# cr1m5onk1ng/text_similarity

Hardware: AMD Instinct MI355X
Metric: sentences/sec encoded + Mpairs/sec cosine top-k @ N=1M d=384 (higher is better)
Workload: dtype bf16 encoder / f16 selection / fp32 scores

## Files before the change

text_similarity_amd/csrc/encoder.hip:

```cpp
#include <math.h>
#include <cmath>

#include <stdlib.h>
#include <string.h>

#include <vector>

#include <type_traits>
#include <utility>

#include "common.h"
#include "gemm_pp.h"

namespace tsim {

__device__ __forceinline__ int64_t packed_off(int64_t t, int f, int W) {
    return ((t >> 5) * (W >> 3) + (f >> 3)) * 256 + (t & 31) * 8 + (f & 7);
}
__device__ __forceinline__ int64_t group_off(int64_t t, int g, int W, int packed) {
    return packed ? packed_off(t, 8 * g, W) * 2 : (t * W + 8 * g) * 2;
}

template <int VPL, bool TYPED = false>
__global__ __launch_bounds__(256) void embed_ln_kernel(const int32_t *__restrict__ ids,
                                                       const int32_t *__restrict__ pos,
                                                       const float *__restrict__ word,
                                                       const float *__restrict__ pos_emb,
                                                       const float *__restrict__ type_tab,
                                                       const float *__restrict__ gamma,
                                                       const float *__restrict__ beta, float eps, int T, int H,
                                                       bf16_t *__restrict__ out, int vocab, int max_pos,
                                                       const int32_t *__restrict__ col, int max_len,
                                                       int *__restrict__ err_flags,
                                                       const int32_t *__restrict__ tok_type = nullptr, int n_types = 0) {
    const int lane = threadIdx.x & 63;
    const int t = blockIdx.x * 4 + (threadIdx.x >> 6);
    if (t >= T) return;
    int id = ids[t], ps = pos[t];
    int ty = 0;
    if constexpr (TYPED) ty = tok_type[t];
    int bad = 0;
    if (id < 0 || id >= vocab) { bad |= TSIM_ENC_ERR_TOKEN_ID; id = id < 0 ? 0 : vocab - 1; }
    if (ps < 0 || ps >= max_pos) { bad |= TSIM_ENC_ERR_POSITION; ps = ps < 0 ? 0 : max_pos - 1; }
    if (col[t] >= max_len || col[t] < 0) bad |= TSIM_ENC_ERR_MAX_LEN;
    if constexpr (TYPED) {
        if (ty < 0 || ty >= n_types) { bad |= TSIM_ENC_ERR_TOKEN_TYPE; ty = ty < 0 ? 0 : n_types - 1; }
    }
    if (bad && lane == 0) atomicOr(err_flags, bad);
    const float *w = word + (int64_t)id * H;
    const float *p = pos_emb + (int64_t)ps * H;
    const float *type_row = TYPED ? type_tab + (int64_t)ty * H : type_tab;
    float v[VPL], pv[VPL], tv[VPL];
#pragma unroll
    for (int i = 0; i < VPL; ++i) {
        v[i] = w[lane + i * 64];
        pv[i] = p[lane + i * 64];
    }
    if (type_row) {
#pragma unroll
        for (int i = 0; i < VPL; ++i) tv[i] = type_row[lane + i * 64];
    }
    float s = 0.f;
#pragma unroll
    for (int i = 0; i < VPL; ++i) {
        float a = v[i];
        if (type_row) a += tv[i];
        a += pv[i];
        v[i] = a;
        s += a;
    }
    const float mean = wave_sum(s) / (float)H;
    float q = 0.f;
#pragma unroll
    for (int i = 0; i < VPL; ++i) {
        const float dlt = v[i] - mean;
        q = fmaf(dlt, dlt, q);
    }
    const float rstd = 1.0f / sqrtf(wave_sum(q) / (float)H + eps);
#pragma unroll
    for (int i = 0; i < VPL; ++i) {
        const int j = lane + i * 64;
        out[(int64_t)t * H + j] = f32_to_bf16((v[i] - mean) * rstd * gamma[j] + beta[j]);
    }
}

enum { EPI_BIAS = 0, EPI_GELU = 1, EPI_RES_LN = 2 };

template <int BM, int BN, int BK, int WAVES_M, int WAVES_N, int NST = 2>
constexpr int gemm_lds_bytes() {
    return NST * (BM + BN) * BK * 2;
}

template <int BM, int BN, int BK, int WAVES_M, int WAVES_N, int EPI, int NST = 2>
__global__ __launch_bounds__(WAVES_M *WAVES_N * 64) void gemm_bf16_kernel(
    const bf16_t *__restrict__ X, const bf16_t *__restrict__ W, const float *__restrict__ bias,
    const bf16_t *__restrict__ res, const float *__restrict__ gamma, const float *__restrict__ beta, float eps,
    bf16_t *__restrict__ out, int M, int N, int K, int mtiles, int ntiles, const bf16_t *__restrict__ Wimg, int xpacked,
    int respacked, int opacked) {
    constexpr int NW = WAVES_M * WAVES_N;
    constexpr int TM = BM / WAVES_M, TN = BN / WAVES_N, MT = TM / 32, NT = TN / 32;
    constexpr int RB = BK * 2;
    constexpr int CPR = RB / 16;
    constexpr int RPS = 256 / RB;
    constexpr int X_BYTES = BM * RB, W_BYTES = BN * RB, STAGE = X_BYTES + W_BYTES;
    constexpr int PIECES = STAGE / 1024, XPIECES = X_BYTES / 1024;
    constexpr int KSTEPS = BK / 16;
    static_assert(TM % 32 == 0 && TN % 32 == 0 && X_BYTES % 1024 == 0 && W_BYTES % 1024 == 0, "tile shape");
    static_assert(NST == 2 || PIECES % NW == 0, "a deep ring needs equal DMA counts per wave");
    constexpr int PPW = (PIECES + NW - 1) / NW;
    extern __shared__ __attribute__((aligned(16))) char smem[];

    const int lane = threadIdx.x & 63;
    const int wave = __builtin_amdgcn_readfirstlane(threadIdx.x >> 6);
    const int wm = wave / WAVES_N, wn = wave % WAVES_N;
    const int r = lane & 31, h = lane >> 5;

    const int b = blockIdx.x, xcd = b & 7, jj = b >> 3;
    const int nt_id = jj % ntiles;
    const int mt_id = (jj / ntiles) * 8 + xcd;
// ... 583 lines not shown
    for (; kt + LR_NST <= nk; kt += LR_NST)
        ff_static_for(std::make_integer_sequence<int, LR_NST>{}, [&](auto sc) __attribute__((always_inline)) {
            do_tile(kt + decltype(sc)::value, sc);
        });
    ff_static_for(std::make_integer_sequence<int, LR_NST - 1>{}, [&](auto sc) __attribute__((always_inline)) {
        if (kt + decltype(sc)::value < nk) do_tile(kt + decltype(sc)::value, sc);
    });
    wait_vmcnt<0>();

    const int64_t m = m0 + wave * 32 + r;
    const bool live = m < M;
    const int64_t mr = live ? m : M - 1;
    const uint32_t ro = (uint32_t)group_off(mr, h, N, respacked), rgs = (uint32_t)group_off(0, 1, N, respacked);
#pragma unroll
    for (int t = 0; t < 12; ++t)
#pragma unroll
        for (int gq = 0; gq < 4; gq += 2) {
            const uint4 o = *reinterpret_cast<const uint4 *>(reinterpret_cast<const char *>(res) + (ro + (4 * t + gq) * rgs));
            auto s0 = __builtin_amdgcn_permlane32_swap(o.x, o.z, false, false);
            auto s1 = __builtin_amdgcn_permlane32_swap(o.y, o.w, false, false);
            const uint32_t a0 = s0[0], c0 = s0[1], a1 = s1[0], c1 = s1[1];
            acc[t][4 * gq + 0] += __uint_as_float(a0 << 16);
            acc[t][4 * gq + 1] += __uint_as_float(a0 & 0xffff0000u);
            acc[t][4 * gq + 2] += __uint_as_float(a1 << 16);
            acc[t][4 * gq + 3] += __uint_as_float(a1 & 0xffff0000u);
            acc[t][4 * gq + 4] += __uint_as_float(c0 << 16);
            acc[t][4 * gq + 5] += __uint_as_float(c0 & 0xffff0000u);
            acc[t][4 * gq + 6] += __uint_as_float(c1 << 16);
            acc[t][4 * gq + 7] += __uint_as_float(c1 & 0xffff0000u);
        }
    float mean, rstd;
#pragma unroll
    for (int pass = 0; pass < 2; ++pass) {
        float tot = 0.f;
#pragma unroll
        for (int w = 0; w < 4; ++w) {
            float sg = 0.f;
#pragma unroll
            for (int t = 3 * w; t < 3 * w + 3; ++t)
#pragma unroll
                for (int q = 0; q < 16; ++q) {
                    if (pass == 0) {
                        sg += acc[t][q];
                    } else {
                        const float dlt = acc[t][q] - mean;
                        sg = fmaf(dlt, dlt, sg);
                    }
                }
            sg += __shfl_xor(sg, 32, 64);
            tot += sg;
        }
        if (pass == 0)
            mean = tot / (float)N;
        else
            rstd = 1.0f / sqrtf(tot / (float)N + eps);
    }
    const uint32_t oo = (uint32_t)group_off(m, h, N, opacked), ogs = (uint32_t)group_off(0, 1, N, opacked);
#pragma unroll
    for (int t = 0; t < 12; ++t) {
        uint32_t pk[8];
#pragma unroll
        for (int gq = 0; gq < 4; ++gq) {
            const int n = 32 * t + 8 * gq + 4 * h;
            const f32x4 gv = *reinterpret_cast<const f32x4 *>(gamma + n), bv = *reinterpret_cast<const f32x4 *>(beta + n);
            const float o0 = fmaf((acc[t][4 * gq + 0] - mean) * rstd, gv[0], bv[0]);
            const float o1 = fmaf((acc[t][4 * gq + 1] - mean) * rstd, gv[1], bv[1]);
            const float o2 = fmaf((acc[t][4 * gq + 2] - mean) * rstd, gv[2], bv[2]);
            const float o3 = fmaf((acc[t][4 * gq + 3] - mean) * rstd, gv[3], bv[3]);
            pk[2 * gq] = pack_bf16x2(o0, o1);
            pk[2 * gq + 1] = pack_bf16x2(o2, o3);
        }
#pragma unroll
        for (int gq = 0; gq < 4; gq += 2) {
            auto s0 = __builtin_amdgcn_permlane32_swap(pk[2 * gq], pk[2 * gq + 2], false, false);
            auto s1w = __builtin_amdgcn_permlane32_swap(pk[2 * gq + 1], pk[2 * gq + 3], false, false);
            if (live)
                *reinterpret_cast<uint4 *>(reinterpret_cast<char *>(out) + (oo + (4 * t + gq) * ogs)) = make_uint4(s0[0], s1w[0], s0[1], s1w[1]);
        }
    }
}

template <int DH, bool REL, bool PK = false>
__global__ __launch_bounds__(256) __attribute__((amdgpu_waves_per_eu(DH <= 32 ? 6 : 4))) void attention_kernel(const bf16_t *__restrict__ qkv,
                                                        const int32_t *__restrict__ cu, const int32_t *__restrict__ col,
                                                        const float *__restrict__ relb, int relw, int H,
                                                        int heads, float scale, bf16_t *__restrict__ ctx, int B, int xcd_map) {
    constexpr int KS = DH / 16;
    constexpr int OT = (DH + 31) / 32;
    constexpr int ROWB = DH * 2 < 64 ? 64 : DH * 2;
    __shared__ __attribute__((aligned(16))) char vimg[4 * 32 * ROWB];
    typedef __attribute__((ext_vector_type(4))) short s16x4;
    const int lane = threadIdx.x & 63;
    const int wave = __builtin_amdgcn_readfirstlane(threadIdx.x >> 6);
    int seq = blockIdx.x;
    if (xcd_map) {
        seq = (blockIdx.x & 7) * (gridDim.x >> 3) + (blockIdx.x >> 3);
        if (seq >= B) return;
    }
    const int head = blockIdx.y * 4 + wave, qb = blockIdx.z;
    const int t0 = cu[seq], S = cu[seq + 1] - t0;
    if (qb * 32 >= S || head >= heads) return;
    const int r = lane & 31, h = lane >> 5;
    const int64_t H3 = 3 * (int64_t)H;
    const int qi = qb * 32 + r;
    const int tq = t0 + (qi < S ? qi : S - 1);

    bf16x8 qf[KS];
    {
        const bf16_t *qp = PK ? qkv + packed_off(tq, head * DH + 8 * h, (int)H3) : qkv + tq * H3 + head * DH + 8 * h;
#pragma unroll
        for (int s = 0; s < KS; ++s) {
            qf[s] = *reinterpret_cast<const bf16x8 *>(qp + (PK ? 2 * 256 : 16) * s);
        }
    }
    const int qcol = REL ? col[tq] : 0;
    f32x16 o[OT];
#pragma unroll
    for (int ob = 0; ob < OT; ++ob)
#pragma unroll
        for (int g = 0; g < 16; ++g) o[ob][g] = 0.f;
    float m = -INFINITY, l = 0.f;

    for (int k0 = 0; k0 < S; k0 += 32) {
        const int kr = k0 + r;
        const int tk = t0 + (kr < S ? kr : S - 1);
        f32x16 sc;
#pragma unroll
        for (int g = 0; g < 16; ++g) sc[g] = 0.f;
        constexpr int CH = DH / 16;
        uint4 vr[CH];
        {
            const bf16_t *kp = PK ? qkv + packed_off(tk, H + head * DH + 8 * h, (int)H3) : qkv + tk * H3 + H + head * DH + 8 * h;
            const bf16_t *vsrc = PK ? qkv + packed_off(tk, 2 * H + head * DH + h * (DH / 2), (int)H3)
                                    : qkv + tk * H3 + 2 * H + head * DH + h * (DH / 2);
            bf16x8 kf[KS];
#pragma unroll
            for (int s = 0; s < KS; ++s) kf[s] = *reinterpret_cast<const bf16x8 *>(kp + (PK ? 2 * 256 : 16) * s);
#pragma unroll
            for (int c = 0; c < CH; ++c) vr[c] = *reinterpret_cast<const uint4 *>(vsrc + (PK ? 256 : 8) * c);
#pragma unroll
            for (int s = 0; s < KS; ++s) sc = __builtin_amdgcn_mfma_f32_32x32x16_bf16(kf[s], qf[s], sc, 0, 0, 0);
        }
        float bm = -INFINITY;
#pragma unroll
        for (int g = 0; g < 16; ++g) {
            const int key = k0 + (g & 3) + 8 * (g >> 2) + 4 * h;
            float v = sc[g] * scale;
            if (REL) {
                const int kc = col[t0 + (key < S ? key : S - 1)];
                v += relb[head * relw + (kc - qcol) + (relw >> 1)];
            }
            v = key < S ? v : -INFINITY;
            sc[g] = v;
            bm = fmaxf(bm, v);
        }
        bm = fmaxf(bm, __shfl_xor(bm, 32, 64));
        const float mn = fmaxf(m, bm);
        const float corr = __expf(m - mn);
        float ps = 0.f;
#pragma unroll
        for (int g = 0; g < 16; ++g) {
            sc[g] = __expf(sc[g] - mn);
            ps += sc[g];
        }
        ps += __shfl_xor(ps, 32, 64);
        l = l * corr + ps;
        m = mn;
#pragma unroll
        for (int ob = 0; ob < OT; ++ob)
#pragma unroll
            for (int g = 0; g < 16; ++g) o[ob][g] *= corr;
        bf16x8 pf[2];
#pragma unroll
        for (int s = 0; s < 2; ++s)
#pragma unroll
            for (int j = 0; j < 8; ++j) pf[s][j] = (__bf16)sc[8 * s + j];
        {
            char *vrow = vimg + wave * (32 * ROWB) + r * ROWB + h * DH;
#pragma unroll
            for (int c = 0; c < CH; ++c) *reinterpret_cast<uint4 *>(vrow + 16 * c) = vr[c];
        }
        __builtin_amdgcn_wave_barrier();
#pragma unroll
        for (int ob = 0; ob < OT; ++ob) {
// ... 391 lines not shown
                    const double de = (double)(float)hv - (double)y[j] * inv;
                    r2 = fma(de, de, r2);
                }
                unit[(int64_t)b * ld_unit + j] = hv;
            }
            if (rho_max) {
                const float rho = rho_round_up(sqrt(wave_sum_f64(r2)));
                if (lane == 0) rho_publish(rho_max, rho);
            }
        }
    }
}

static int dense_rows_launch(const float *x, int B, int d_in, const float *w, const float *bias, int d_out, int act, int normalize,
                             float *out, unit_t *unit, int ld_unit, float *rho_max, hipStream_t st) {
    if (B <= 0) return TSIM_OK;
    const dim3 grid((unsigned)((B + DN_ROWS - 1) / DN_ROWS));
    const size_t lds = (size_t)DN_ROWS * d_out * sizeof(float);
#define DENSE(NT) hipLaunchKernelGGL(dense_rows_kernel<NT>, grid, dim3(64 * DN_WAVES), lds, st, x, B, d_in, w, bias, d_out, act, normalize, out, unit, ld_unit, rho_max)
    const int nt = ((d_out + 15) / 16 + DN_WAVES - 1) / DN_WAVES;
    if (nt <= 1) DENSE(1); else if (nt <= 2) DENSE(2); else if (nt <= 3) DENSE(3); else if (nt <= 4) DENSE(4);
    else if (nt <= 6) DENSE(6); else DENSE(8);
#undef DENSE
    TSIM_HIP_CHECK(hipGetLastError());
    return TSIM_OK;
}

static int dense_check(int d_in, int d_out, int act, const float *w) {
    TSIM_REQUIRE(d_in >= 8 && d_in <= DN_MAX && d_in % 8 == 0, "dense: d_in=%d outside [8, %d] or not a multiple of 8", d_in, DN_MAX);
    TSIM_REQUIRE(d_out >= 8 && d_out <= DN_MAX && d_out % 8 == 0, "dense: d_out=%d outside [8, %d] or not a multiple of 8", d_out,
                 DN_MAX);
    TSIM_REQUIRE(w || d_out == d_in, "dense: without a weight matrix d_out (%d) must equal d_in (%d)", d_out, d_in);
    TSIM_REQUIRE(act == TSIM_ACT_IDENTITY || act == TSIM_ACT_TANH, "dense: unknown activation %d (TSIM_ACT_IDENTITY, TSIM_ACT_TANH)",
                 act);
    TSIM_REQUIRE(((uintptr_t)w & 15) == 0, "dense: the weight matrix must be 16-byte aligned");
    return TSIM_OK;
}

static uint16_t host_f32_to_bf16(float f) {
    uint32_t u;
    memcpy(&u, &f, 4);
    if ((u & 0x7fffffffu) > 0x7f800000u) return (uint16_t)((u >> 16) | 0x40);
    u += 0x7fffu + ((u >> 16) & 1u);
    return (uint16_t)(u >> 16);
}

struct DevBuf {
    void *p = nullptr;
    ~DevBuf() {
        if (p) (void)hipFree(p);
    }
};

}

using namespace tsim;

struct tsim_encoder {
    tsim_encoder_config cfg;
    int Tp = 0;
    float *word = nullptr, *pos = nullptr, *type0 = nullptr, *emb_g = nullptr, *emb_b = nullptr, *relb = nullptr;
    int relw = 0;
    int n_types = 0;
    float *head_wpT = nullptr, *head_bp = nullptr, *head_wc = nullptr, *head_bc = nullptr;
    int n_labels = 0;
    int head_act = TSIM_ACT_TANH;
    struct Layer {
        bf16_t *wqkv, *wo, *w1, *w2;
        bf16_t *pqkv = nullptr, *po = nullptr;
        bf16_t *lo = nullptr, *l2 = nullptr;
        bf16_t *lo32 = nullptr, *l232 = nullptr;
        uint8_t *qqkv = nullptr, *qo = nullptr, *q1 = nullptr, *q2 = nullptr;
        uint8_t *sqkv = nullptr, *so = nullptr, *s1 = nullptr, *s2 = nullptr;
        float *bqkv, *bo, *b1, *b2, *g1, *be1, *g2, *be2;
    };
    std::vector<Layer> layers;
    std::vector<void *> allocs;
    bf16_t *x0 = nullptr, *x1 = nullptr, *qkv = nullptr, *ctx = nullptr, *h1 = nullptr;
    float *ybuf = nullptr;
    float *lnimg = nullptr;
    float *head_x = nullptr;
    uint8_t *aq = nullptr, *as = nullptr, *hq = nullptr, *hs = nullptr;
    int *err_flags = nullptr;
};

namespace tsim {

static int dev_alloc(tsim_encoder *e, size_t bytes, void **out) {
    void *p = nullptr;
    hipError_t err = hipMalloc(&p, bytes);
    if (err != hipSuccess) return fail(TSIM_ENOMEM, "hipMalloc(%zu) failed: %s", bytes, hipGetErrorString(err));
    e->allocs.push_back(p);
    *out = p;
    return TSIM_OK;
}

static int upload_f32(tsim_encoder *e, const float *h, size_t n, float **out) {
    int rc = dev_alloc(e, n * 4, (void **)out);
    if (rc) return rc;
    TSIM_HIP_CHECK(hipMemcpy(*out, h, n * 4, hipMemcpyHostToDevice));
    return TSIM_OK;
}

static int upload_bf16(tsim_encoder *e, const std::vector<const float *> &parts, size_t n_each, bf16_t **out) {
    std::vector<uint16_t> tmp(n_each * parts.size());
    for (size_t p = 0; p < parts.size(); ++p)
        for (size_t i = 0; i < n_each; ++i) tmp[p * n_each + i] = host_f32_to_bf16(parts[p][i]);
    int rc = dev_alloc(e, tmp.size() * 2, (void **)out);
    if (rc) return rc;
    TSIM_HIP_CHECK(hipMemcpy(*out, tmp.data(), tmp.size() * 2, hipMemcpyHostToDevice));
    return TSIM_OK;
}

static uint8_t host_f32_to_e4m3(float v) {
    const uint8_t sign = std::signbit(v) ? 0x80 : 0;
    const double a = std::fabs((double)v);
    if (a == 0.0) return sign;
    int exp;
    const double mant = std::frexp(a, &exp);
    long byte;
    if (a >= std::ldexp(1.0, -6))
        byte = ((long)(exp - 1 + 7) << 3) + std::lrint((mant * 2.0 - 1.0) * 8.0);
    else
        byte = std::lrint(std::ldexp(a, 9));
    if (byte > 0x7e) byte = 0x7e;
    return (uint8_t)byte | sign;
}

static int upload_mxfp8(tsim_encoder *e, const std::vector<const float *> &parts, size_t n_rows, size_t K, uint8_t **q,
                        uint8_t **sc) {
    const size_t rows = n_rows * parts.size(), nb = K / 32;
    std::vector<uint8_t> hq(rows * K), hs(rows * nb);
    for (size_t p = 0; p < parts.size(); ++p)
        for (size_t r = 0; r < n_rows; ++r)
            for (size_t b = 0; b < nb; ++b) {
                const float *src = parts[p] + r * K + b * 32;
                float amax = 0.f;
                for (int i = 0; i < 32; ++i) amax = std::fmax(amax, std::fabs(src[i]));
                int sexp = 0;
                if (amax > 0.f) {
                    int ex;
                    (void)std::frexp((double)amax, &ex);
                    sexp = ex - 1 - 8;
                    sexp = sexp < -127 ? -127 : (sexp > 127 ? 127 : sexp);
                }
                uint8_t *dst = hq.data() + (p * n_rows + r) * K + b * 32;
                for (int i = 0; i < 32; ++i) {
                    double y = std::ldexp((double)src[i], -sexp);
                    y = y > 448.0 ? 448.0 : (y < -448.0 ? -448.0 : y);
                    dst[i] = host_f32_to_e4m3((float)y);
                }
                hs[(p * n_rows + r) * nb + b] = (uint8_t)(sexp + 127);
            }
    int rc = dev_alloc(e, hq.size(), (void **)q);
    if (rc) return rc;
    if ((rc = dev_alloc(e, hs.size(), (void **)sc))) return rc;
    TSIM_HIP_CHECK(hipMemcpy(*q, hq.data(), hq.size(), hipMemcpyHostToDevice));
    TSIM_HIP_CHECK(hipMemcpy(*sc, hs.data(), hs.size(), hipMemcpyHostToDevice));
    return TSIM_OK;
}

static int mpnet_bucket(int rel, int num_buckets) {
    int ret = 0;
    int n = -rel;
    const int nb = num_buckets / 2;
    if (n < 0) {
// ... 390 lines not shown
    }
    e->layers.resize(L);
    for (int l = 0; l < L; ++l) {
        const tsim_layer_weights_host &lw = w->layers[l];
        tsim_encoder::Layer &d = e->layers[l];
        if ((rc = upload_bf16(e, {lw.wq, lw.wk, lw.wv}, (size_t)H * H, &d.wqkv))) return bail(rc);
        if ((rc = upload_bf16(e, {lw.wo}, (size_t)H * H, &d.wo))) return bail(rc);
        if ((rc = upload_bf16(e, {lw.w1}, (size_t)F * H, &d.w1))) return bail(rc);
        if ((rc = upload_bf16(e, {lw.w2}, (size_t)H * F, &d.w2))) return bail(rc);
        if (mx) {
            if ((rc = upload_mxfp8(e, {lw.wq, lw.wk, lw.wv}, H, H, &d.qqkv, &d.sqkv))) return bail(rc);
            if ((rc = upload_mxfp8(e, {lw.wo}, H, H, &d.qo, &d.so))) return bail(rc);
            if ((rc = upload_mxfp8(e, {lw.w1}, F, H, &d.q1, &d.s1))) return bail(rc);
            if ((rc = upload_mxfp8(e, {lw.w2}, H, F, &d.q2, &d.s2))) return bail(rc);
        }
        auto repack = [&](const void *src, int n_rows, int kbytes, void **dst) {
            int r2 = dev_alloc(e, (size_t)n_rows * kbytes, dst);
            return r2 ? r2 : pack_w(src, *dst, n_rows, kbytes, gemm_pp_tile_width(n_rows), nullptr);
        };
        if (mx) {
            void *t;
            if ((rc = repack(d.qqkv, 3 * H, H, &t))) return bail(rc); d.qqkv = (uint8_t *)t;
            if ((rc = repack(d.qo, H, H, &t))) return bail(rc); d.qo = (uint8_t *)t;
            if ((rc = repack(d.q1, F, H, &t))) return bail(rc); d.q1 = (uint8_t *)t;
            if ((rc = repack(d.q2, H, F, &t))) return bail(rc); d.q2 = (uint8_t *)t;
        } else if (H >= 512 && H % 256 == 0 && gemm_pp_supported(H, H) && gemm_pp_supported(F, H) && gemm_pp_supported(H, F)) {
            if ((rc = repack(d.wqkv, 3 * H, H * 2, (void **)&d.pqkv))) return bail(rc);
            if ((rc = repack(d.wo, H, H * 2, (void **)&d.po))) return bail(rc);
        }
        if (!mx && H == 384 && F % 64 == 0) {
            if ((rc = dev_alloc(e, (size_t)H * H * 2, (void **)&d.lo))) return bail(rc);
            if ((rc = dev_alloc(e, (size_t)H * F * 2, (void **)&d.l2))) return bail(rc);
            hipLaunchKernelGGL(pack_gemm_w_kernel, dim3((unsigned)((H * H / 8 + 255) / 256)), dim3(256), 0, 0,
                               reinterpret_cast<const uint4 *>(d.wo), reinterpret_cast<uint4 *>(d.lo), 384, 64, H);
            hipLaunchKernelGGL(pack_gemm_w_kernel, dim3((unsigned)((H * F / 8 + 255) / 256)), dim3(256), 0, 0,
                               reinterpret_cast<const uint4 *>(d.w2), reinterpret_cast<uint4 *>(d.l2), 384, 64, F);
            if ((rc = dev_alloc(e, (size_t)H * H * 2, (void **)&d.lo32))) return bail(rc);
            if ((rc = dev_alloc(e, (size_t)H * F * 2, (void **)&d.l232))) return bail(rc);
            hipLaunchKernelGGL(pack_frag_w_kernel, dim3((unsigned)((H * H / 8 + 255) / 256)), dim3(256), 0, 0,
                               reinterpret_cast<const uint4 *>(d.wo), reinterpret_cast<uint4 *>(d.lo32), 384, H);
            hipLaunchKernelGGL(pack_frag_w_kernel, dim3((unsigned)((H * F / 8 + 255) / 256)), dim3(256), 0, 0,
                               reinterpret_cast<const uint4 *>(d.w2), reinterpret_cast<uint4 *>(d.l232), 384, F);
            if (hipGetLastError() != hipSuccess) return bail(fail(TSIM_EHIP, "LayerNorm GEMM weight packing failed"));
        }
        std::vector<float> bq(3 * (size_t)H);
        memcpy(bq.data(), lw.bq, H * 4);
        memcpy(bq.data() + H, lw.bk, H * 4);
        memcpy(bq.data() + 2 * H, lw.bv, H * 4);
        if ((rc = upload_f32(e, bq.data(), bq.size(), &d.bqkv))) return bail(rc);
        if ((rc = upload_f32(e, lw.bo, H, &d.bo))) return bail(rc);
        if ((rc = upload_f32(e, lw.b1, F, &d.b1))) return bail(rc);
        if ((rc = upload_f32(e, lw.b2, H, &d.b2))) return bail(rc);
        if ((rc = upload_f32(e, lw.ln1_g, H, &d.g1))) return bail(rc);
        if ((rc = upload_f32(e, lw.ln1_b, H, &d.be1))) return bail(rc);
        if ((rc = upload_f32(e, lw.ln2_g, H, &d.g2))) return bail(rc);
        if ((rc = upload_f32(e, lw.ln2_b, H, &d.be2))) return bail(rc);
    }
    const size_t Tp = e->Tp;
    struct { bf16_t **p; size_t n; } acts[] = {{&e->x0, Tp * H}, {&e->x1, Tp * H}, {&e->qkv, Tp * 3 * H},
                                               {&e->ctx, Tp * H}, {&e->h1, Tp * F}};
    for (auto &a : acts) {
        if ((rc = dev_alloc(e, a.n * 2, (void **)a.p))) return bail(rc);
        if (hipMemset(*a.p, 0, a.n * 2) != hipSuccess) return bail(fail(TSIM_EHIP, "hipMemset failed"));
    }
    if (H >= 512 && H % 256 == 0 && gemm_pp_supported(H, H)) {
        if ((rc = dev_alloc(e, Tp * H * 4, (void **)&e->ybuf))) return bail(rc);
        if (hipMemset(e->ybuf, 0, Tp * H * 4) != hipSuccess) return bail(fail(TSIM_EHIP, "hipMemset failed"));
    }
    if (!mx && H == 384 && F % 64 == 0) {
        const size_t blocks = (Tp + 31) / 32 < (size_t)LS_MAX_BLOCKS ? (Tp + 31) / 32 : (size_t)LS_MAX_BLOCKS;
        const size_t bytes = blocks * 4 * 12 * 64 * 16;
        if ((rc = dev_alloc(e, bytes, (void **)&e->lnimg))) return bail(rc);
        if (hipMemset(e->lnimg, 0, bytes) != hipSuccess) return bail(fail(TSIM_EHIP, "hipMemset failed"));
    }
    if ((size_t)cfg->max_seqs * H * 4 > Tp * 3 * H * 2 && (rc = dev_alloc(e, (size_t)cfg->max_seqs * H * 4, (void **)&e->head_x)))
        return bail(rc);
    if (mx) {
        struct { uint8_t **p; size_t n; } qb[] = {{&e->aq, Tp * H}, {&e->as, Tp * H / 32}, {&e->hq, Tp * F}, {&e->hs, Tp * F / 32}};
        for (auto &a : qb) {
            if ((rc = dev_alloc(e, a.n, (void **)a.p))) return bail(rc);
            if (hipMemset(*a.p, 0, a.n) != hipSuccess) return bail(fail(TSIM_EHIP, "hipMemset failed"));
        }
    }
    if ((rc = dev_alloc(e, 256, (void **)&e->err_flags))) return bail(rc);
    if (hipMemset(e->err_flags, 0, 256) != hipSuccess) return bail(fail(TSIM_EHIP, "hipMemset failed"));
    if (hipDeviceSynchronize() != hipSuccess) return bail(fail(TSIM_EHIP, "sync after upload failed"));
    *out = e;
    return TSIM_OK;
}

extern "C" int tsim_encoder_error_flags(tsim_encoder *e, int32_t *flags_host, void *stream) {
    TSIM_REQUIRE(e && flags_host, "encoder_error_flags: null pointer");
    hipStream_t st = reinterpret_cast<hipStream_t>(stream);
    TSIM_HIP_CHECK(hipMemcpyAsync(flags_host, e->err_flags, 4, hipMemcpyDeviceToHost, st));
    TSIM_HIP_CHECK(hipMemsetAsync(e->err_flags, 0, 4, st));
    TSIM_HIP_CHECK(hipStreamSynchronize(st));
    return TSIM_OK;
}

extern "C" int tsim_quantize_mxfp8(const void *x_bf16, int64_t rows, int K, void *q_out, void *scale_out, void *stream) {
    TSIM_REQUIRE(x_bf16 && q_out && scale_out, "quantize_mxfp8: null pointer");
    TSIM_REQUIRE(rows >= 0 && K > 0, "quantize_mxfp8: bad shape rows=%lld K=%d", (long long)rows, K);
    return quant_mx(static_cast<const bf16_t *>(x_bf16), rows, K, static_cast<uint8_t *>(q_out),
                    static_cast<uint8_t *>(scale_out), reinterpret_cast<hipStream_t>(stream));
}

extern "C" int tsim_gemm_mxfp8(const void *xq, const void *xs, const void *wq, const void *ws, const float *bias,
                               float *out_f32, int M, int N, int K, void *stream) {
    TSIM_REQUIRE(xq && xs && wq && ws && bias && out_f32, "gemm_mxfp8: null pointer");
    TSIM_REQUIRE(M >= 0 && N > 0 && K > 0, "gemm_mxfp8: bad shape M=%d N=%d K=%d", M, N, K);
    return gemm_pp_mx(PP_EPI_F32, static_cast<const uint8_t *>(xq), static_cast<const uint8_t *>(xs),
                      static_cast<const uint8_t *>(wq), 0, static_cast<const uint8_t *>(ws), bias, out_f32, nullptr, M, N, K,
                      reinterpret_cast<hipStream_t>(stream));
}

#ifdef TSIM_PP_STAMPS
extern "C" int tsim_debug_xr_stamps(unsigned long long *out16, int reset) {
    if (hipMemcpyFromSymbol(out16, HIP_SYMBOL(tsim::g_xr_stamps), 128) != hipSuccess) return 1;
    if (reset) { unsigned long long z[16] = {0}; if (hipMemcpyToSymbol(HIP_SYMBOL(tsim::g_xr_stamps), z, 128) != hipSuccess) return 1; }
    return 0;
}
#endif

extern "C" void tsim_encoder_destroy(tsim_encoder *e) {
    if (!e) return;
    for (void *p : e->allocs) (void)hipFree(p);
    delete e;
}

extern "C" int tsim_encoder_set_token_types(tsim_encoder *e, const float *type_emb_host, int32_t n_types) {
    TSIM_REQUIRE(e && type_emb_host, "encoder_set_token_types: null pointer");
    TSIM_REQUIRE(e->cfg.arch != TSIM_ARCH_MPNET, "encoder_set_token_types: BERT only (MPNet has no token-type table)");
    TSIM_REQUIRE(n_types >= 1, "encoder_set_token_types: n_types=%d < 1", n_types);
    float *tab = nullptr;
    if (int rc = upload_f32(e, type_emb_host, (size_t)n_types * e->cfg.hidden, &tab)) return rc;
    e->type0 = tab;
    e->n_types = n_types;
    return TSIM_OK;
}

extern "C" int tsim_encoder_set_cls_head(tsim_encoder *e, const float *pool_w_host, const float *pool_b_host,
                                         const float *cls_w_host, const float *cls_b_host, int32_t num_labels) {
    return tsim_encoder_set_cls_head_act(e, pool_w_host, pool_b_host, cls_w_host, cls_b_host, num_labels, TSIM_ACT_TANH);
}

extern "C" int tsim_encoder_set_cls_head_act(tsim_encoder *e, const float *pool_w_host, const float *pool_b_host,
                                             const float *cls_w_host, const float *cls_b_host, int32_t num_labels, int32_t act) {
    TSIM_REQUIRE(e && pool_w_host && pool_b_host && cls_w_host && cls_b_host, "encoder_set_cls_head: null pointer");
    TSIM_REQUIRE(e->cfg.arch != TSIM_ARCH_MPNET, "encoder_set_cls_head: BERT only");
    TSIM_REQUIRE(act == TSIM_ACT_TANH || act == TSIM_ACT_RELU, "encoder_set_cls_head: activation %d (TSIM_ACT_TANH, TSIM_ACT_RELU)", act);
    TSIM_REQUIRE(num_labels >= 1 && num_labels <= CLS_MAX_LABELS, "encoder_set_cls_head: num_labels=%d outside [1, %d]", num_labels,
                 CLS_MAX_LABELS);
    const int H = e->cfg.hidden;
    TSIM_REQUIRE(H % 64 == 0 && H <= CLS_WIDE_H, "encoder_set_cls_head: hidden=%d unsupported", H);
    std::vector<float> wT((size_t)H * H);
    for (int o = 0; o < H; ++o)
        for (int k = 0; k < H; ++k) wT[(size_t)k * H + o] = pool_w_host[(size_t)o * H + k];
    int rc;
    if ((rc = upload_f32(e, wT.data(), wT.size(), &e->head_wpT))) return rc;
    if ((rc = upload_f32(e, pool_b_host, H, &e->head_bp))) return rc;
    if ((rc = upload_f32(e, cls_w_host, (size_t)num_labels * H, &e->head_wc))) return rc;
    if ((rc = upload_f32(e, cls_b_host, num_labels, &e->head_bc))) return rc;
    e->n_labels = num_labels;
    e->head_act = act;
    return TSIM_OK;
}

extern "C" int tsim_encoder_forward(tsim_encoder *e, const int32_t *tok_ids, const int32_t *tok_pos,
                                    const int32_t *tok_col, const int32_t *cu_seqlens, int32_t T, int32_t B,
                                    int32_t max_len, float *pooled_f32, void *unit_bf16, int ld_unit, float *unit_rho_max,
                                    void *last_hidden_bf16, void *stream) {
    return tsim_encoder_forward_ex(e, tok_ids, nullptr, tok_pos, tok_col, cu_seqlens, T, B, max_len, pooled_f32, unit_bf16, ld_unit,
                                   unit_rho_max, last_hidden_bf16, nullptr, stream);
}

extern "C" int tsim_encoder_forward_ex(tsim_encoder *e, const int32_t *tok_ids, const int32_t *tok_type, const int32_t *tok_pos,
                                       const int32_t *tok_col, const int32_t *cu_seqlens, int32_t T, int32_t B,
                                       int32_t max_len, float *pooled_f32, void *unit_bf16, int ld_unit, float *unit_rho_max,
                                       void *last_hidden_bf16, float *logits_f32, void *stream) {
    TSIM_REQUIRE(e && cu_seqlens && (T == 0 || (tok_ids && tok_pos)), "encoder_forward: null pointer");
    TSIM_REQUIRE(!tok_type || e->n_types > 0, "encoder_forward: tok_type given but no token-type table was set "
                 "(tsim_encoder_set_token_types)");
    TSIM_REQUIRE(!logits_f32 || e->n_labels > 0, "encoder_forward: logits requested but no classification head was set "
                 "(tsim_encoder_set_cls_head)");
    TSIM_REQUIRE(T >= 0 && B >= 0 && T <= e->cfg.max_tokens && B <= e->cfg.max_seqs,
                 "encoder_forward: T=%d B=%d exceed capacity (%d tokens, %d sequences)", T, B, e->cfg.max_tokens, e->cfg.max_seqs);
    const int pos_span = max_len + (e->cfg.arch != TSIM_ARCH_BERT ? e->cfg.pad_id + 1 : 0);
    TSIM_REQUIRE(max_len >= 0 && pos_span <= e->cfg.max_pos,
                 "encoder_forward: sequences of %d tokens need position rows up to %d, the table has %d", max_len, pos_span - 1,
                 e->cfg.max_pos);
    TSIM_REQUIRE(!unit_bf16 || ld_unit >= e->cfg.hidden, "encoder_forward: ld_unit < hidden");
    TSIM_REQUIRE(!unit_bf16 || e->cfg.hidden <= 768, "encoder_forward: unit rows need a width <= 768 (got %d)", e->cfg.hidden);
    if (B == 0) return TSIM_OK;
    hipStream_t st = reinterpret_cast<hipStream_t>(stream);
    const tsim_encoder_config &c = e->cfg;
    const int H = c.hidden, F = c.ffn, dh = H / c.heads;
    const bool mx = c.weight_dtype == TSIM_W_MXFP8;
    int rc;
    if (T > 0) {
        const unsigned g = (unsigned)((T + 3) / 4);
        const int32_t *colp = tok_col ? tok_col : tok_pos;
        const int col_limit = tok_col || c.arch == TSIM_ARCH_BERT ? max_len : c.max_pos;
#define EMBED(V) hipLaunchKernelGGL(embed_ln_kernel<V>, dim3(g), dim3(256), 0, st, tok_ids, tok_pos, e->word, e->pos, e->type0, e->emb_g, e->emb_b, c.ln_eps, T, H, e->x0, c.vocab, c.max_pos, colp, col_limit, e->err_flags, nullptr, 0)
#define EMBED_T(V) hipLaunchKernelGGL((embed_ln_kernel<V, true>), dim3(g), dim3(256), 0, st, tok_ids, tok_pos, e->word, e->pos, e->type0, e->emb_g, e->emb_b, c.ln_eps, T, H, e->x0, c.vocab, c.max_pos, colp, col_limit, e->err_flags, tok_type, e->n_types)
        if (tok_type) {
            if (H == 64) EMBED_T(1); else if (H == 384) EMBED_T(6); else if (H == 768) EMBED_T(12); else EMBED_T(16);
        } else if (H == 64) EMBED(1); else if (H == 384) EMBED(6); else if (H == 768) EMBED(12); else EMBED(16);
#undef EMBED_T
#undef EMBED
        TSIM_HIP_CHECK(hipGetLastError());
        const float scale = 1.0f / sqrtf((float)dh);
        const bool rel = c.arch == TSIM_ARCH_MPNET;
        const bool pk = !mx && !rel && use_packed_layout(H, F);
        const int32_t *col = rel ? (tok_col ? tok_col : tok_pos) : nullptr;
        const int qblocks = (max_len + 31) / 32 > 0 ? (max_len + 31) / 32 : 1;
        const dim3 agrid((unsigned)(((B + 7) / 8) * 8), (unsigned)((c.heads + 3) / 4), (unsigned)qblocks);
        for (int l = 0; l < c.num_layers; ++l) {
            const tsim_encoder::Layer &L = e->layers[l];
            const bool x0pk = pk && l > 0, x0pk_next = pk && l + 1 < c.num_layers;
            if (mx) {
                if (l == 0 && (rc = quant_mx(e->x0, T, H, e->aq, e->as, st))) return rc;
                if ((rc = gemm_pp_mx(PP_EPI_BIAS, e->aq, e->as, L.qqkv, 1, L.sqkv, L.bqkv, e->qkv, nullptr, T, 3 * H, H, st))) return rc;
            } else if (pk) {
                rc = x0pk ? gemm_xres2<EPI_BIAS, true, true>(e->x0, L.wqkv, L.bqkv, e->qkv, T, 3 * H, st)
                          : gemm_xres2<EPI_BIAS, true>(e->x0, L.wqkv, L.bqkv, e->qkv, T, 3 * H, st);
                if (rc) return rc;
            } else if ((rc = gemm_plain<EPI_BIAS>(e->x0, L.wqkv, L.pqkv, L.bqkv, e->qkv, T, 3 * H, H, st))) return rc;
#define ATT(D)                                                                                                 \
    do {                                                                                                       \
        if (rel)                                                                                               \
            hipLaunchKernelGGL((attention_kernel<D, true>), agrid, dim3(256), 0, st, e->qkv, cu_seqlens, col,  \
                               e->relb, e->relw, H, c.heads, scale, e->ctx, B, 1);                                         \
        else if (pk)                                                                                           \
            hipLaunchKernelGGL((attention_kernel<D, false, true>), agrid, dim3(256), 0, st, e->qkv, cu_seqlens, col, \
                               e->relb, e->relw, H, c.heads, scale, e->ctx, B, 1);                                         \
        else                                                                                                   \
            hipLaunchKernelGGL((attention_kernel<D, false>), agrid, dim3(256), 0, st, e->qkv, cu_seqlens, col, \
                               e->relb, e->relw, H, c.heads, scale, e->ctx, B, 1);                                         \
    } while (0)
            if (dh == 16) ATT(16); else if (dh == 32) ATT(32); else ATT(64);
#undef ATT
            TSIM_HIP_CHECK(hipGetLastError());
            if (mx) {
                if ((rc = quant_mx(e->ctx, T, H, e->aq, e->as, st))) return rc;
                if ((rc = gemm_pp_mx(PP_EPI_F32, e->aq, e->as, L.qo, 1, L.so, L.bo, e->ybuf, nullptr, T, H, H, st))) return rc;
                if ((rc = res_ln_rows(e->ybuf, e->x0, L.g1, L.be1, c.ln_eps, e->x1, e->aq, e->as, T, H, st))) return rc;
                if ((rc = gemm_pp_mx(PP_EPI_GELU_MX, e->aq, e->as, L.q1, 1, L.s1, L.b1, e->hq, e->hs, T, F, H, st))) return rc;
                if ((rc = gemm_pp_mx(PP_EPI_F32, e->hq, e->hs, L.q2, 1, L.s2, L.b2, e->ybuf, nullptr, T, H, F, st))) return rc;
                if ((rc = res_ln_rows(e->ybuf, e->x1, L.g2, L.be2, c.ln_eps, e->x0, e->aq, e->as, T, H, st))) return rc;
                continue;
            }
            if ((rc = gemm_res_ln(e->ctx, L.wo, L.po, L.bo, e->x0, L.g1, L.be1, c.ln_eps, e->x1, T, H, H, e->ybuf, st, L.lo, L.lo32, false, e->lnimg, x0pk, pk))) return rc;
            if (pk) {
                if ((rc = gemm_xres2<EPI_GELU, true, true>(e->x1, L.w1, L.b1, e->h1, T, F, st))) return rc;
            } else if ((rc = gemm_plain<EPI_GELU>(e->x1, L.w1, nullptr, L.b1, e->h1, T, F, H, st))) return rc;
            if ((rc = gemm_res_ln(e->h1, L.w2, nullptr, L.b2, e->x1, L.g2, L.be2, c.ln_eps, e->x0, T, H, F, e->ybuf, st, L.l2, L.l232, pk, e->lnimg, pk, x0pk_next))) return rc;
        }
        if (last_hidden_bf16)
            TSIM_HIP_CHECK(hipMemcpyAsync(last_hidden_bf16, e->x0, (size_t)T * H * 2, hipMemcpyDeviceToDevice, st));
    }
    if (pooled_f32 || unit_bf16) {
        const unsigned g = (unsigned)((B + 3) / 4);
#define POOL(V) hipLaunchKernelGGL(pool_packed_kernel<V>, dim3(g), dim3(256), 0, st, e->x0, cu_seqlens, B, H, pooled_f32, (unit_t *)unit_bf16, ld_unit, unit_bf16 ? unit_rho_max : nullptr)
        if (H % 8 != 0 || H > 1024 || (unit_bf16 && ld_unit % 8 != 0))
            return fail(TSIM_EUNSUPPORTED, "encoder: pooling needs a hidden size that is a multiple of 8, at most 1024 (got %d)", H);
        if (((uintptr_t)pooled_f32 | (uintptr_t)unit_bf16) & 15)
            return fail(TSIM_EINVAL, "encoder: pooled / unit outputs must be 16-byte aligned");
        if (H <= 512) POOL(1); else POOL(2);
#undef POOL
        TSIM_HIP_CHECK(hipGetLastError());
    }
    if (logits_f32) {
        const dim3 cgrid((unsigned)((B + CLS_ROWS - 1) / CLS_ROWS)), cblock((unsigned)H);
#define CLS_WIDE(MAXH, ACT)                                                                                       \
    hipLaunchKernelGGL((cls_head_wide_kernel<MAXH, ACT>), cgrid, cblock, 0, st, e->x0, cu_seqlens, B, H, e->head_wpT, \
                       e->head_bp, e->head_wc, e->head_bc, e->n_labels, logits_f32)
        if (e->head_act == TSIM_ACT_RELU) {
            if (H <= CLS_MAX_H) CLS_WIDE(CLS_MAX_H, TSIM_ACT_RELU); else CLS_WIDE(CLS_WIDE_H, TSIM_ACT_RELU);
        } else if (H <= CLS_MAX_H) {
            hipLaunchKernelGGL(cls_head_kernel, cgrid, cblock, 0, st, e->x0, cu_seqlens,
                               B, H, e->head_wpT, e->head_bp, e->head_wc, e->head_bc, e->n_labels, logits_f32);
        } else CLS_WIDE(CLS_WIDE_H, TSIM_ACT_TANH);
#undef CLS_WIDE
        TSIM_HIP_CHECK(hipGetLastError());
    }
    return TSIM_OK;
}

extern "C" int tsim_encoder_forward_head(tsim_encoder *e, const int32_t *tok_ids, const int32_t *tok_type, const int32_t *tok_pos,
                                         const int32_t *tok_col, const int32_t *cu_seqlens, int32_t T, int32_t B, int32_t max_len,
                                         const tsim_sentence_head *head, float *emb_f32, void *unit_f16, int ld_unit,
                                         float *unit_rho_max, void *last_hidden_bf16, void *stream) {
    if (!head)
        return tsim_encoder_forward_ex(e, tok_ids, tok_type, tok_pos, tok_col, cu_seqlens, T, B, max_len, emb_f32, unit_f16, ld_unit,
                                       unit_rho_max, last_hidden_bf16, nullptr, stream);
    TSIM_REQUIRE(e, "encoder_forward_head: null encoder");
    const int H = e->cfg.hidden, mode = head->pool_mode, d_out = head->d_out;
    TSIM_REQUIRE(mode >= TSIM_POOL_MEAN && mode <= TSIM_POOL_MEAN_SQRT_LEN, "encoder_forward_head: unknown pool_mode %d", mode);
    TSIM_REQUIRE(head->normalize == 0 || head->normalize == 1, "encoder_forward_head: normalize=%d is not 0 / 1", head->normalize);
    TSIM_REQUIRE(d_out >= 0, "encoder_forward_head: d_out=%d < 0", d_out);
    if (d_out) {
        TSIM_REQUIRE(head->dense_w, "encoder_forward_head: d_out=%d without dense_w", d_out);
        if (int rc = dense_check(H, d_out, head->dense_act, head->dense_w)) return rc;
    } else {
        TSIM_REQUIRE(!head->dense_w && !head->dense_b, "encoder_forward_head: dense weights given with d_out = 0");
    }
    const int width = d_out ? d_out : H;
    TSIM_REQUIRE(!unit_f16 || width <= 768, "encoder_forward_head: unit rows need a final width <= 768 (got %d)", width);
    TSIM_REQUIRE(!unit_f16 || (ld_unit >= width && ld_unit % 8 == 0), "encoder_forward_head: ld_unit=%d (final width %d)", ld_unit,
                 width);
    TSIM_REQUIRE(H % 8 == 0 && H <= 1024, "encoder_forward_head: pooling needs hidden %% 8 == 0 and <= 1024 (got %d)", H);
    TSIM_REQUIRE((((uintptr_t)emb_f32 | (uintptr_t)unit_f16) & 15) == 0, "encoder_forward_head: outputs must be 16-byte aligned");
    if (int rc = tsim_encoder_forward_ex(e, tok_ids, tok_type, tok_pos, tok_col, cu_seqlens, T, B, max_len, nullptr, nullptr, 0,
                                         nullptr, last_hidden_bf16, nullptr, stream))
        return rc;
    if (B == 0 || (!emb_f32 && !unit_f16)) return TSIM_OK;
    hipStream_t st = reinterpret_cast<hipStream_t>(stream);
    float *px = d_out ? (e->head_x ? e->head_x : reinterpret_cast<float *>(e->qkv)) : emb_f32;
    unit_t *pu = d_out ? nullptr : static_cast<unit_t *>(unit_f16);
    const bool norm = !d_out && head->normalize;
    const unsigned g = (unsigned)((B + 3) / 4);
// ... 27 lines not shown
```

Measured before the change: 874,200.

## Launch attention over compacted per-sequence query-block work items

Block 0 of the embedding kernel now builds a compact list of (sequence start, length, query block) items using a block-wide prefix scan over cu_seqlens. The attention grid is sized by the item count instead of B×max query blocks, so blocks that used to exit early on short sequences are no longer launched. This adds a serial scan in one block of the embed kernel, an extra buffer, and an indirection load in attention. It also removes the old sequence-to-XCD mapping in favour of an item-to-XCD striping.

Result: no change. 882,600, median of 6 (+1.0%).

```diff
diff --git a/text_similarity_amd/csrc/encoder.hip b/text_similarity_amd/csrc/encoder.hip
--- a/text_similarity_amd/csrc/encoder.hip
+++ b/text_similarity_amd/csrc/encoder.hip
@@ -19,6 +19,45 @@
 }
 __device__ __forceinline__ int64_t group_off(int64_t t, int g, int W, int packed) {
     return packed ? packed_off(t, 8 * g, W) * 2 : (t * W + 8 * g) * 2;
+}
+
+constexpr int ATT_ITEM_SEQS = 4;
+
+__device__ __forceinline__ void build_attention_items(const int32_t *__restrict__ cu, int B, int qblocks, int4 *__restrict__ items,
+                                                      int cap) {
+    __shared__ int wsum[4];
+    const int tid = threadIdx.x, lane = tid & 63, wave = tid >> 6;
+    int carry = 0;
+    for (int c0 = 0; c0 < B; c0 += 256 * ATT_ITEM_SEQS) {
+        const int s0 = c0 + tid * ATT_ITEM_SEQS;
+        int c[ATT_ITEM_SEQS + 1], n[ATT_ITEM_SEQS], tot = 0;
+#pragma unroll
+        for (int j = 0; j <= ATT_ITEM_SEQS; ++j) c[j] = cu[s0 + j < B ? s0 + j : B];
+#pragma unroll
+        for (int j = 0; j < ATT_ITEM_SEQS; ++j) {
+            const int S = c[j + 1] - c[j];
+            const int nb = S > 0 ? (S + 31) >> 5 : 0;
+            n[j] = nb < qblocks ? nb : qblocks;
+            tot += n[j];
+        }
+        int inc = tot;
+#pragma unroll
+        for (int d = 1; d < 64; d <<= 1) {
+            const int v = __shfl_up(inc, d, 64);
+            if (lane >= d) inc += v;
+        }
+        if (lane == 63) wsum[wave] = inc;
+        __syncthreads();
+        int base = carry + inc - tot;
+        for (int w = 0; w < wave; ++w) base += wsum[w];
+        carry += wsum[0] + wsum[1] + wsum[2] + wsum[3];
+        __syncthreads();
+#pragma unroll
+        for (int j = 0; j < ATT_ITEM_SEQS; ++j)
+            for (int qb = 0; qb < n[j]; ++qb, ++base)
+                if (base < cap) items[1 + base] = make_int4(c[j], c[j + 1] - c[j], qb, s0 + j);
+    }
+    if (tid == 0) items[0] = make_int4(carry < cap ? carry : cap, 0, 0, 0);
 }
 
 template <int VPL, bool TYPED = false>
@@ -32,9 +71,15 @@
                                                        bf16_t *__restrict__ out, int vocab, int max_pos,
                                                        const int32_t *__restrict__ col, int max_len,
                                                        int *__restrict__ err_flags,
+                                                       const int32_t *__restrict__ cu, int B, int qblocks,
+                                                       int4 *__restrict__ items, int item_cap,
                                                        const int32_t *__restrict__ tok_type = nullptr, int n_types = 0) {
+    if (blockIdx.x == 0) {
+        build_attention_items(cu, B, qblocks, items, item_cap);
+        return;
+    }
     const int lane = threadIdx.x & 63;
-    const int t = blockIdx.x * 4 + (threadIdx.x >> 6);
+    const int t = (blockIdx.x - 1) * 4 + (threadIdx.x >> 6);
     if (t >= T) return;
     int id = ids[t], ps = pos[t];
     int ty = 0;
@@ -784,9 +829,9 @@
 
 template <int DH, bool REL, bool PK = false>
 __global__ __launch_bounds__(256) __attribute__((amdgpu_waves_per_eu(DH <= 32 ? 6 : 4))) void attention_kernel(const bf16_t *__restrict__ qkv,
-                                                        const int32_t *__restrict__ cu, const int32_t *__restrict__ col,
+                                                        const int4 *__restrict__ items, const int32_t *__restrict__ col,
                                                         const float *__restrict__ relb, int relw, int H,
-                                                        int heads, float scale, bf16_t *__restrict__ ctx, int B, int xcd_map) {
+                                                        int heads, float scale, bf16_t *__restrict__ ctx) {
     constexpr int KS = DH / 16;
     constexpr int OT = (DH + 31) / 32;
     constexpr int ROWB = DH * 2 < 64 ? 64 : DH * 2;
@@ -794,14 +839,14 @@
     typedef __attribute__((ext_vector_type(4))) short s16x4;
     const int lane = threadIdx.x & 63;
     const int wave = __builtin_amdgcn_readfirstlane(threadIdx.x >> 6);
-    int seq = blockIdx.x;
-    if (xcd_map) {
-        seq = (blockIdx.x & 7) * (gridDim.x >> 3) + (blockIdx.x >> 3);
-        if (seq >= B) return;
-    }
-    const int head = blockIdx.y * 4 + wave, qb = blockIdx.z;
-    const int t0 = cu[seq], S = cu[seq + 1] - t0;
-    if (qb * 32 >= S || head >= heads) return;
+    const int n_items = items[0].x;
+    const int nx = (n_items + 7) >> 3, slot = blockIdx.x >> 3;
+    const int it = (blockIdx.x & 7) * nx + slot;
+    if (slot >= nx || it >= n_items) return;
+    const int4 item = items[1 + it];
+    const int head = blockIdx.y * 4 + wave;
+    const int t0 = item.x, S = item.y, qb = item.z;
+    if (head >= heads) return;
     const int r = lane & 31, h = lane >> 5;
     const int64_t H3 = 3 * (int64_t)H;
     const int qi = qb * 32 + r;
@@ -1359,6 +1404,8 @@
     float *head_x = nullptr;
     uint8_t *aq = nullptr, *as = nullptr, *hq = nullptr, *hs = nullptr;
     int *err_flags = nullptr;
+    int4 *att_items = nullptr;
+    int att_item_cap = 0;
 };
 
 namespace tsim {
@@ -1915,6 +1962,9 @@
             if (hipMemset(*a.p, 0, a.n) != hipSuccess) return bail(fail(TSIM_EHIP, "hipMemset failed"));
         }
     }
+    e->att_item_cap = cfg->max_seqs + cfg->max_tokens / 32 + 8;
+    if ((rc = dev_alloc(e, ((size_t)e->att_item_cap + 1) * sizeof(int4), (void **)&e->att_items))) return bail(rc);
+    if (hipMemset(e->att_items, 0, ((size_t)e->att_item_cap + 1) * sizeof(int4)) != hipSuccess) return bail(fail(TSIM_EHIP, "hipMemset failed"));
     if ((rc = dev_alloc(e, 256, (void **)&e->err_flags))) return bail(rc);
     if (hipMemset(e->err_flags, 0, 256) != hipSuccess) return bail(fail(TSIM_EHIP, "hipMemset failed"));
     if (hipDeviceSynchronize() != hipSuccess) return bail(fail(TSIM_EHIP, "sync after upload failed"));
@@ -2031,11 +2081,12 @@
     const bool mx = c.weight_dtype == TSIM_W_MXFP8;
     int rc;
     if (T > 0) {
-        const unsigned g = (unsigned)((T + 3) / 4);
+        const unsigned g = (unsigned)((T + 3) / 4) + 1;
+        const int qblocks = (max_len + 31) / 32 > 0 ? (max_len + 31) / 32 : 1;
         const int32_t *colp = tok_col ? tok_col : tok_pos;
         const int col_limit = tok_col || c.arch == TSIM_ARCH_BERT ? max_len : c.max_pos;
-#define EMBED(V) hipLaunchKernelGGL(embed_ln_kernel<V>, dim3(g), dim3(256), 0, st, tok_ids, tok_pos, e->word, e->pos, e->type0, e->emb_g, e->emb_b, c.ln_eps, T, H, e->x0, c.vocab, c.max_pos, colp, col_limit, e->err_flags, nullptr, 0)
-#define EMBED_T(V) hipLaunchKernelGGL((embed_ln_kernel<V, true>), dim3(g), dim3(256), 0, st, tok_ids, tok_pos, e->word, e->pos, e->type0, e->emb_g, e->emb_b, c.ln_eps, T, H, e->x0, c.vocab, c.max_pos, colp, col_limit, e->err_flags, tok_type, e->n_types)
+#define EMBED(V) hipLaunchKernelGGL(embed_ln_kernel<V>, dim3(g), dim3(256), 0, st, tok_ids, tok_pos, e->word, e->pos, e->type0, e->emb_g, e->emb_b, c.ln_eps, T, H, e->x0, c.vocab, c.max_pos, colp, col_limit, e->err_flags, cu_seqlens, B, qblocks, e->att_items, e->att_item_cap, nullptr, 0)
+#define EMBED_T(V) hipLaunchKernelGGL((embed_ln_kernel<V, true>), dim3(g), dim3(256), 0, st, tok_ids, tok_pos, e->word, e->pos, e->type0, e->emb_g, e->emb_b, c.ln_eps, T, H, e->x0, c.vocab, c.max_pos, colp, col_limit, e->err_flags, cu_seqlens, B, qblocks, e->att_items, e->att_item_cap, tok_type, e->n_types)
         if (tok_type) {
             if (H == 64) EMBED_T(1); else if (H == 384) EMBED_T(6); else if (H == 768) EMBED_T(12); else EMBED_T(16);
         } else if (H == 64) EMBED(1); else if (H == 384) EMBED(6); else if (H == 768) EMBED(12); else EMBED(16);
@@ -2046,8 +2097,9 @@
         const bool rel = c.arch == TSIM_ARCH_MPNET;
         const bool pk = !mx && !rel && use_packed_layout(H, F);
         const int32_t *col = rel ? (tok_col ? tok_col : tok_pos) : nullptr;
-        const int qblocks = (max_len + 31) / 32 > 0 ? (max_len + 31) / 32 : 1;
-        const dim3 agrid((unsigned)(((B + 7) / 8) * 8), (unsigned)((c.heads + 3) / 4), (unsigned)qblocks);
+        const int64_t by_tokens = (int64_t)B + T / 32, by_len = (int64_t)B * qblocks;
+        const int64_t item_bound = by_tokens < by_len ? by_tokens : by_len;
+        const dim3 agrid((unsigned)((item_bound + 7) / 8 * 8), (unsigned)((c.heads + 3) / 4));
         for (int l = 0; l < c.num_layers; ++l) {
             const tsim_encoder::Layer &L = e->layers[l];
             const bool x0pk = pk && l > 0, x0pk_next = pk && l + 1 < c.num_layers;
@@ -2062,14 +2114,14 @@
 #define ATT(D)                                                                                                 \
     do {                                                                                                       \
         if (rel)                                                                                               \
-            hipLaunchKernelGGL((attention_kernel<D, true>), agrid, dim3(256), 0, st, e->qkv, cu_seqlens, col,  \
-                               e->relb, e->relw, H, c.heads, scale, e->ctx, B, 1);                                         \
+            hipLaunchKernelGGL((attention_kernel<D, true>), agrid, dim3(256), 0, st, e->qkv, e->att_items, col,  \
+                               e->relb, e->relw, H, c.heads, scale, e->ctx);                                               \
         else if (pk)                                                                                           \
-            hipLaunchKernelGGL((attention_kernel<D, false, true>), agrid, dim3(256), 0, st, e->qkv, cu_seqlens, col, \
-                               e->relb, e->relw, H, c.heads, scale, e->ctx, B, 1);                                         \
+            hipLaunchKernelGGL((attention_kernel<D, false, true>), agrid, dim3(256), 0, st, e->qkv, e->att_items, col, \
+                               e->relb, e->relw, H, c.heads, scale, e->ctx);                                               \
         else                                                                                                   \
-            hipLaunchKernelGGL((attention_kernel<D, false>), agrid, dim3(256), 0, st, e->qkv, cu_seqlens, col, \
-                               e->relb, e->relw, H, c.heads, scale, e->ctx, B, 1);                                         \
+            hipLaunchKernelGGL((attention_kernel<D, false>), agrid, dim3(256), 0, st, e->qkv, e->att_items, col, \
+                               e->relb, e->relw, H, c.heads, scale, e->ctx);                                               \
     } while (0)
             if (dh == 16) ATT(16); else if (dh == 32) ATT(32); else ATT(64);
 #undef ATT
```
